# lbcb-sci/GNNome

Measured on AMD Instinct MI355X. Metric: edges/sec full-graph GatedGCN fwd, higher is better.
Workload: dtype f32

## Files before the change

### gnnome_amd/csrc/common.h

```cpp
#pragma once
#include <hip/hip_runtime.h>
#include <stdint.h>
#include <stdio.h>

#include "../../include/gnnome_hip.h"

namespace gnnome {

void set_error(const char* fmt, ...);

enum { kTuneGateVariant = 0, kTuneGateAblation = 1, kTuneLinearVariant = 2, kTuneGateTileOrder = 3, kTuneGateExperiment = 4, kTuneAggLdsKiB = 5, kTuneAggHubs = 6, kTuneAggVariant = 7, kTuneRefVariant = 8, kTuneOverlapBand = 9, kTuneArith = 10, kTuneCount = 16 };
int tuning(int key);

struct GateEnc {
    const float* e_raw;
    const int32_t* srt_eid;
    const float *W1, *b1, *W2, *b2;
    const float *W23, *b23;
};

struct GateBnBwd {
    const float *a, *c1, *c2, *mean, *rstd, *scale, *shift;
    float* a_out;
    int64_t n_once;
    unsigned* amax_bits = nullptr;
};

struct GateBfArgs {
    const float* e_in;
    float* e_out;
    int64_t E;
    const float* B1h;
    const float* B2h;
    int ldn;
    const int32_t* srt_src;
    const int32_t* srt_dst;
    const float* W3;
    int ldw;
    const float* scale;
    const float* shift;
    float* stats;
    int num_tiles;
    int abl;
    long long* prof;
    int xp;
    int num_cblocks, ld_out;
    GateEnc enc;
    GateBnBwd bnb;
};
int gate_bf_launch(int hidden, int mode, bool enc, const GateBfArgs& args, hipStream_t s, bool x16 = false, int extra = 0);
int gate_stream_launch(const float* e_in, float* e_out, int64_t E, const float* B1h, const float* B2h, int ldn, const int32_t* ss,
                       const int32_t* sd, const float* W3, int ldw, const float* scale, const float* shift, hipStream_t s);

int ws_linear_acc(const float* A, int64_t M, int K, const float* W, int ldw, float* C, hipStream_t s);
int stream_linear_acc_256(const float* A, int64_t M, const float* W, int ldw, float* C, hipStream_t s);
int gate_pl256_launch(int mode, const GateBfArgs& a, hipStream_t s, bool x16 = false);
int gate_f16_launch(int mode, const GateBfArgs& a, int grid, hipStream_t s, bool x16 = false);
int gate_enc256_launch(const GateBfArgs& a, hipStream_t s);
int gate_pl256_stats_rows();
void hub_cache_invalidate();
long long* gate_profile_buffer();
int linear_refm_launch(const float* A, int64_t M, int K, int lda, const float* W, int ldw, const float* bias, int Nout, float* C, int ldc,
                       hipStream_t s);
int gate_refm_launch(int hidden, bool with_enc, const float* e_in, float* e_out, int64_t E, const float* B1h, const float* B2h, int ldn,
                     const int32_t* ss, const int32_t* sd, const float* W3, int ldw, const float* b3, const float* scale, const float* shift,
                     const GateEnc& enc, hipStream_t s);

#define GN_REQUIRE(cond, ...)                 \
    do {                                      \
        if (!(cond)) {                        \
            ::gnnome::set_error(__VA_ARGS__); \
            return GNNOME_EINVAL;             \
        }                                     \
    } while (0)

#define GN_HIP(call)                                                                              \
    do {                                                                                          \
        hipError_t err__ = (call);                                                                \
        if (err__ != hipSuccess) {                                                                \
            ::gnnome::set_error("%s failed: %s (%s:%d)", #call, hipGetErrorString(err__), __FILE__, \
                                __LINE__);                                                        \
            return GNNOME_EHIP;                                                                   \
        }                                                                                         \
    } while (0)

#define GN_LAUNCH_CHECK() GN_HIP(hipGetLastError())

constexpr int kWave = 64;
constexpr int kXcds = 8;
constexpr int kNumCUs = 256;
int persistent_grid();
constexpr float kAggEps = 1e-6f;
constexpr float kNormEps = 1e-5f;

typedef float f32x4 __attribute__((ext_vector_type(4)));
typedef float f32x16 __attribute__((ext_vector_type(16)));

__device__ __forceinline__ unsigned bf16_bits(float x) {
    const unsigned u = __float_as_uint(x);
    return (u + 0x7FFFu + ((u >> 16) & 1u)) >> 16;
}
__device__ __forceinline__ uint2 pack_bf16x4(const f32x4 v) {
    return make_uint2(bf16_bits(v[0]) | (bf16_bits(v[1]) << 16), bf16_bits(v[2]) | (bf16_bits(v[3]) << 16));
}
__device__ __forceinline__ f32x4 unpack_bf16x4(const uint2 p) {
    return f32x4{__uint_as_float(p.x << 16), __uint_as_float(p.x & 0xFFFF0000u), __uint_as_float(p.y << 16),
                 __uint_as_float(p.y & 0xFFFF0000u)};
}
template <bool X16>
__device__ __forceinline__ f32x4 load4_as(const void* base, int64_t off) {
    if (X16) return unpack_bf16x4(*reinterpret_cast<const uint2*>(reinterpret_cast<const uint16_t*>(base) + off));
    return *reinterpret_cast<const f32x4*>(reinterpret_cast<const float*>(base) + off);
}
template <bool X16>
__device__ __forceinline__ void store4_as(void* base, int64_t off, const f32x4 v) {
    if (X16)
        *reinterpret_cast<uint2*>(reinterpret_cast<uint16_t*>(base) + off) = pack_bf16x4(v);
    else
        *reinterpret_cast<f32x4*>(reinterpret_cast<float*>(base) + off) = v;
}


__device__ __forceinline__ int xcd_remap(int bid, int n) {
    const int xcd = bid % kXcds, q = n / kXcds, r = n % kXcds;
    const int base = xcd < r ? xcd * (q + 1) : r * (q + 1) + (xcd - r) * q;
    return base + bid / kXcds;
}

__device__ __forceinline__ float sigmoidf_(float x) { return __builtin_amdgcn_rcpf(1.0f + __expf(-x)); }

__device__ __forceinline__ float relu_keep_nan(float t) { return t < 0.f ? 0.f : t; }

__device__ __forceinline__ void wave_amax_to(unsigned* amax_bits, float v) {
#pragma unroll
    for (int o = 32; o > 0; o >>= 1) v = fmaxf(v, __shfl_xor(v, o));
    if ((threadIdx.x & 63) == 0) {
        const unsigned b = __float_as_uint(v);
        if (b > __hip_atomic_load(amax_bits, __ATOMIC_RELAXED, __HIP_MEMORY_SCOPE_AGENT)) atomicMax(amax_bits, b);
    }
}

__device__ __forceinline__ float half_wave_sum(float v) {
    v += __shfl_xor(v, 1);
    v += __shfl_xor(v, 2);
    v += __shfl_xor(v, 4);
    v += __shfl_xor(v, 8);
    v += __shfl_xor(v, 16);
    return v;
}

}
```

### gnnome_amd/csrc/node_aggregate.hip

```cpp
#include "common.h"

#include <algorithm>
#include <map>
#include <mutex>
#include <utility>

namespace gnnome {

constexpr int kAggThreads = 256;
constexpr int kHubThreshold = 4096;
constexpr int kHubChunks = 128;
constexpr int kHubCap = 64;
constexpr int kHubMaxH = 256;
constexpr int kRecItems = 20;

struct HubScratch {
    const void *key_in = nullptr, *key_out = nullptr;
    int64_t key_n = -1;
    int* count = nullptr;
    int* nodes = nullptr;
    float* partials = nullptr;
    int* host_count = nullptr;
    hipEvent_t ready = nullptr;
    bool pending = false;
    int known = -1;
};

static std::map<std::pair<int, hipStream_t>, HubScratch> g_hub_table;
static std::mutex g_hub_guard;

void hub_cache_invalidate() {
    int dev = 0;
    if (hipGetDevice(&dev) != hipSuccess) return;
    std::lock_guard<std::mutex> lock(g_hub_guard);
    for (auto& kv : g_hub_table) {
        if (kv.first.first != dev) continue;
        kv.second.key_in = kv.second.key_out = nullptr;
        kv.second.key_n = -1;
        kv.second.known = -1;
        kv.second.pending = false;
    }
}

static HubScratch* hub_scratch(hipStream_t s, bool* capturing_unallocated, const void* in_ptr = nullptr, const void* out_ptr = nullptr,
                               int64_t n = -1) {
    int dev = 0;
    if (hipGetDevice(&dev) != hipSuccess) return nullptr;
    auto it = g_hub_table.find(std::make_pair(dev, s));
    if (it == g_hub_table.end() || it->second.partials == nullptr) {
        hipStreamCaptureStatus st = hipStreamCaptureStatusNone;
        if (hipStreamIsCapturing(s, &st) == hipSuccess && st != hipStreamCaptureStatusNone) {
            for (auto& kv : g_hub_table) {
                const HubScratch& h = kv.second;
                if (kv.first.first == dev && h.partials != nullptr && h.key_n == n &&
                    ((h.key_in == in_ptr && h.key_out == out_ptr) || (h.key_in == out_ptr && h.key_out == in_ptr)))
                    return &kv.second;
            }
            for (auto& kv : g_hub_table)
                if (kv.first.first == dev && kv.second.partials != nullptr) return &kv.second;
            *capturing_unallocated = true;
            return nullptr;
        }
    }
    HubScratch& h = g_hub_table[std::make_pair(dev, s)];
    if (h.partials == nullptr) {
        if (h.count == nullptr && hipMalloc(&h.count, sizeof(int) * (1 + kHubCap)) != hipSuccess) return nullptr;
        h.nodes = h.count + 1;
        if (hipMalloc(&h.partials, sizeof(float) * (size_t)kHubCap * kHubChunks * 4 * kHubMaxH) != hipSuccess) return nullptr;
        if (hipHostMalloc(&h.host_count, sizeof(int), hipHostMallocDefault) != hipSuccess) h.host_count = nullptr;
        if (h.host_count && hipEventCreateWithFlags(&h.ready, hipEventDisableTiming) != hipSuccess) h.ready = nullptr;
    }
    return &h;
}

__device__ __forceinline__ int hub_key(int node) { return 0x7fffffff - node; }
__device__ __forceinline__ int hub_node_at(const int* __restrict__ nodes, int slot) { return 0x7fffffff - nodes[slot]; }

__global__ __launch_bounds__(256) void k_find_hubs(const int32_t* __restrict__ in_ptr, const int32_t* __restrict__ out_ptr, int64_t n,
                                                   int* __restrict__ count, int* __restrict__ nodes) {
    const int64_t i = (int64_t)blockIdx.x * 256 + threadIdx.x;
    if (i >= n) return;
    const int cnt = (in_ptr[i + 1] - in_ptr[i]) + (out_ptr[i + 1] - out_ptr[i]);
    if (cnt > kHubThreshold) {
        atomicAdd(count, 1);
        int key = hub_key((int)i);
        if (key < __hip_atomic_load(nodes + kHubCap - 1, __ATOMIC_RELAXED, __HIP_MEMORY_SCOPE_AGENT)) return;
        for (int slot = 0; slot < kHubCap && key != 0; ++slot) {
            const int old = atomicMax(nodes + slot, key);
            key = min(old, key);
        }
    }
}

template <int H>
__device__ __forceinline__ float group_sum(float v) {
    constexpr int LPR = H / 4;
#pragma unroll
    for (int m = LPR; m < 64; m <<= 1) v += __shfl_xor(v, m);
    return v;
}

template <int H>
__device__ __forceinline__ float row_sum(float v) {
    constexpr int LPR = H / 4;
#pragma unroll
    for (int m = 1; m < LPR; m <<= 1) v += __shfl_xor(v, m);
    return v;
}

template <int H, int U = (H == 256 ? 8 : 4)>
__device__ __forceinline__ void accumulate_items(const float* __restrict__ e, const float* __restrict__ A2h, const float* __restrict__ A3h,
                                                 int ldn, const int32_t* __restrict__ srt_src, const int32_t* __restrict__ out_pos,
                                                 const int32_t* __restrict__ out_dst, int ib, int din, int ob, int lo, int hi, int lane,
                                                 int group, int c, f32x4& nf, f32x4& df, f32x4& nb, f32x4& db) {
    constexpr int LPR = H / 4, G = 64 / LPR;
    for (int base = lo; base < hi; base += 64) {
        const int j = base + lane;
        int my_p = 0, my_n = 0;
        if (j < din) {
            my_p = ib + j;
            my_n = srt_src[my_p];
        } else if (j < hi) {
            my_p = out_pos[ob + j - din];
            my_n = out_dst[ob + j - din];
        }
        const int m = min(64, hi - base);
        for (int j0 = 0; j0 < m; j0 += G * U) {
            f32x4 x[U], a[U];
            bool live[U], fwd[U];
#pragma unroll
            for (int u = 0; u < U; ++u) {
                const int item = j0 + u * G + group;
                live[u] = item < m;
                const int it = live[u] ? item : 0;
                const int p = __shfl(my_p, it), nn = __shfl(my_n, it);
                fwd[u] = base + it < din;
                const float* tb = fwd[u] ? A2h : A3h;
                x[u] = *reinterpret_cast<const f32x4*>(e + (int64_t)p * H + c);
                a[u] = *reinterpret_cast<const f32x4*>(tb + (int64_t)nn * ldn + c);
            }
#pragma unroll
            for (int u = 0; u < U; ++u) {
                if (live[u]) {
                    f32x4 s;
#pragma unroll
                    for (int k = 0; k < 4; ++k) s[k] = sigmoidf_(x[u][k]);
                    if (fwd[u]) {
                        nf += s * a[u];
                        df += s;
                    } else {
                        nb += s * a[u];
                        db += s;
                    }
                }
            }
        }
    }
}

template <int H, int U = (H == 256 ? 8 : 4), bool NOBR = false, bool NTOUT = false, bool TBLFIX = false>
__device__ __forceinline__ void accumulate_items_split(const float* __restrict__ e, const float* __restrict__ A2h, const float* __restrict__ A3h,
                                                       int ldn, const int32_t* __restrict__ srt_src, const int32_t* __restrict__ out_pos,
                                                       const int32_t* __restrict__ out_dst, int ib, int din, int ob, int lo, int hi, int lane,
                                                       int group, int c, f32x4& nf, f32x4& df, f32x4& nb, f32x4& db, int recv = 0,
                                                       bool rec_small = false) {
    constexpr int LPR = H / 4, G = 64 / LPR;
    for (int base = lo; base < hi; base += 64) {
        const int j = base + lane;
        int my_p = 0, my_n = 0;
        if (rec_small) {
            const int jo = min(max(j - din, 0), kRecItems - 1);
            my_n = __shfl(recv, j < din ? 4 + min(j, kRecItems - 1) : 4 + 2 * kRecItems + jo);
            my_p = __shfl(recv, 4 + kRecItems + jo);
        } else if (j < din) {
            my_n = srt_src[ib + j];
        } else if (j < hi) {
            my_p = out_pos[ob + j - din];
            my_n = out_dst[ob + j - din];
        }
        const int m = min(64, hi - base);
        const int m_in = min(m, max(din - base, 0));
        for (int j0 = 0; j0 < m_in; j0 += G * U) {
            f32x4 x[U], a[U];
            bool live[U];
#pragma unroll
            for (int u = 0; u < U; ++u) {
                const int item = j0 + u * G + group;
                live[u] = item < m_in;
                x[u] = *reinterpret_cast<const f32x4*>(e + (int64_t)(ib + base + (live[u] ? item : 0)) * H + c);
            }
#pragma unroll
            for (int u = 0; u < U; ++u) {
                const int item = j0 + u * G + group;
                const int nn = TBLFIX ? (ib & 1023) : __shfl(my_n, live[u] ? item : 0);
                a[u] = *reinterpret_cast<const f32x4*>(A2h + (int64_t)nn * ldn + c);
            }
#pragma unroll
            for (int u = 0; u < U; ++u) {
                if (NOBR) {
                    f32x4 s;
#pragma unroll
                    for (int k = 0; k < 4; ++k) s[k] = live[u] ? sigmoidf_(x[u][k]) : 0.f;
                    nf += s * a[u];
                    df += s;
                } else if (live[u]) {
                    f32x4 s;
#pragma unroll
                    for (int k = 0; k < 4; ++k) s[k] = sigmoidf_(x[u][k]);
                    nf += s * a[u];
                    df += s;
                }
            }
        }
        for (int j0 = m_in / (G * U) * (G * U); j0 < m; j0 += G * U) {
            f32x4 x[U], a[U];
            bool live[U];
#pragma unroll
            for (int u = 0; u < U; ++u) {
                const int item = j0 + u * G + group;
                live[u] = item >= m_in && item < m;
                const int it = live[u] ? item : m_in;
                const int p = __shfl(my_p, it), nn = TBLFIX ? (ib & 1023) : __shfl(my_n, it);
                x[u] = NTOUT ? __builtin_nontemporal_load(reinterpret_cast<const f32x4*>(e + (int64_t)p * H + c))
                             : *reinterpret_cast<const f32x4*>(e + (int64_t)p * H + c);
                a[u] = *reinterpret_cast<const f32x4*>(A3h + (int64_t)nn * ldn + c);
            }
#pragma unroll
            for (int u = 0; u < U; ++u) {
                if (NOBR) {
                    f32x4 s;
#pragma unroll
                    for (int k = 0; k < 4; ++k) s[k] = live[u] ? sigmoidf_(x[u][k]) : 0.f;
                    nb += s * a[u];
                    db += s;
                } else if (live[u]) {
                    f32x4 s;
#pragma unroll
                    for (int k = 0; k < 4; ++k) s[k] = sigmoidf_(x[u][k]);
                    nb += s * a[u];
                    db += s;
                }
            }
        }
    }
}

template <int H>
__global__ __launch_bounds__(kAggThreads) void k_hub_partials(const float* __restrict__ e, const float* __restrict__ A2h,
                                                              const float* __restrict__ A3h, int ldn, const int32_t* __restrict__ in_ptr,
                                                              const int32_t* __restrict__ srt_src, const int32_t* __restrict__ out_ptr,
                                                              const int32_t* __restrict__ out_pos, const int32_t* __restrict__ out_dst,
                                                              int64_t n_out, const int* __restrict__ hub_count,
                                                              const int* __restrict__ hub_nodes, float* __restrict__ partials) {
    constexpr int LPR = H / 4;
    const int lane = threadIdx.x & 63, wave = threadIdx.x >> 6;
    const int ch = blockIdx.x * (kAggThreads / 64) + wave;
    const int group = lane / LPR, c = (lane % LPR) * 4;
    const int nh = min(*hub_count, kHubCap);
    for (int h = 0; h < nh; ++h) {
        const int64_t node = hub_node_at(hub_nodes, h);
        if (node >= n_out) continue;
        const int ib = in_ptr[node], din = in_ptr[node + 1] - ib;
        const int ob = out_ptr[node], cnt = din + out_ptr[node + 1] - ob;
        const int per = ((cnt + kHubChunks - 1) / kHubChunks + 63) / 64 * 64;
        const int lo = min(cnt, ch * per), hi = min(cnt, lo + per);
        f32x4 nf = {0.f, 0.f, 0.f, 0.f}, df = nf, nb = nf, db = nf;
        accumulate_items<H>(e, A2h, A3h, ldn, srt_src, out_pos, out_dst, ib, din, ob, lo, hi, lane, group, c, nf, df, nb, db);
        f32x4 o0, o1, o2, o3;
#pragma unroll
        for (int k = 0; k < 4; ++k) {
            o0[k] = group_sum<H>(nf[k]);
            o1[k] = group_sum<H>(df[k]);
            o2[k] = group_sum<H>(nb[k]);
            o3[k] = group_sum<H>(db[k]);
        }
        if (group == 0) {
            float* pp = partials + ((int64_t)h * kHubChunks + ch) * 4 * H + c;
            *reinterpret_cast<f32x4*>(pp) = o0;
            *reinterpret_cast<f32x4*>(pp + H) = o1;
            *reinterpret_cast<f32x4*>(pp + 2 * H) = o2;
            *reinterpret_cast<f32x4*>(pp + 3 * H) = o3;
        }
    }
}

template <int H, int NORM, int MODE, bool HUBFIN = false, int U = (H == 256 ? 8 : 4), int WPS = 0, int SPLIT = 0, bool REC = false>
__global__ __launch_bounds__(kAggThreads, (WPS > 0 ? WPS : 1)) void k_node_aggregate(
    const float* __restrict__ e, int64_t n_out, const float* __restrict__ A1h, const float* __restrict__ A2h,
    const float* __restrict__ A3h, int ldn, const int32_t* __restrict__ in_ptr, const int32_t* __restrict__ srt_src,
    const int32_t* __restrict__ out_ptr, const int32_t* __restrict__ out_pos, const int32_t* __restrict__ out_dst,
    const float* __restrict__ h_in, int ldh, float* __restrict__ h_out, const float* __restrict__ scale,
    const float* __restrict__ shift, int total_blocks, float* __restrict__ aux0, float* __restrict__ aux1,
    float* __restrict__ aux2, float* __restrict__ aux3, const int* __restrict__ hub_count, const int* __restrict__ hub_nodes,
    const float* __restrict__ hub_partials, int64_t node0, int norm_width, const int32_t* __restrict__ records = nullptr) {
    constexpr int LPR = H / 4;
    const int lane = threadIdx.x & 63, wave = threadIdx.x >> 6;
    int64_t node;
    int hub_slot = -1;
    if (HUBFIN) {
        hub_slot = blockIdx.x * (kAggThreads / 64) + wave;
        if (hub_slot >= min(*hub_count, kHubCap)) return;
        node = hub_node_at(hub_nodes, hub_slot);
    } else {
        node = node0 + (int64_t)xcd_remap(blockIdx.x, total_blocks) * (kAggThreads / 64) + wave;
    }
    if (node >= n_out) return;
    const int group = lane / LPR, c = (lane % LPR) * 4;

    int ib, din, ob, cnt, recv = 0;
    if (REC) {
        recv = records[node * 64 + lane];
        ib = __builtin_amdgcn_readlane(recv, 0), din = __builtin_amdgcn_readlane(recv, 1);
        ob = __builtin_amdgcn_readlane(recv, 2), cnt = din + __builtin_amdgcn_readlane(recv, 3);
    } else {
        ib = in_ptr[node], din = in_ptr[node + 1] - ib;
        ob = out_ptr[node], cnt = din + out_ptr[node + 1] - ob;
    }
    const bool rec_small = REC && din <= kRecItems && cnt - din <= kRecItems;
    if (HUBFIN) {
        if (cnt <= kHubThreshold) return;
    } else if (cnt > kHubThreshold && hub_nodes != nullptr) {
        const int nh = min(*hub_count, kHubCap);
        bool listed = false;
        for (int base = 0; base < nh; base += 64) listed |= __ballot(base + lane < nh && hub_nodes[base + lane] == hub_key((int)node)) != 0;
        if (listed) return;
    }
    f32x4 a1 = {0.f, 0.f, 0.f, 0.f};
    if (MODE != 2) a1 = *reinterpret_cast<const f32x4*>(A1h + node * ldn + c);

    f32x4 nf = {0.f, 0.f, 0.f, 0.f}, df = nf, nb = nf, db = nf;
    if (HUBFIN) {
        if (group == 0) {
            const float* pp = hub_partials + ((int64_t)hub_slot * kHubChunks) * 4 * H + c;
            for (int ch = 0; ch < kHubChunks; ++ch, pp += 4 * H) {
                nf += *reinterpret_cast<const f32x4*>(pp);
                df += *reinterpret_cast<const f32x4*>(pp + H);
                nb += *reinterpret_cast<const f32x4*>(pp + 2 * H);
                db += *reinterpret_cast<const f32x4*>(pp + 3 * H);
            }
        }
    } else {
        if (SPLIT == 2)
            accumulate_items_split<H, U>(e, A2h, A3h, ldn, srt_src, out_pos, out_dst, ib, 0, ob, 0, cnt - din, lane, group, c, nf, df, nb, db);
        else if (SPLIT == 4)
            accumulate_items_split<H, U, false, true>(e, A2h, A3h, ldn, srt_src, out_pos, out_dst, ib, din, ob, 0, cnt, lane, group, c, nf, df, nb, db);
        else if (SPLIT == 5)
            accumulate_items_split<H, U, false, false, true>(e, A2h, A3h, ldn, srt_src, out_pos, out_dst, ib, din, ob, 0, cnt, lane, group, c, nf, df, nb, db);
        else if (SPLIT == 3)
            accumulate_items_split<H, U, true>(e, A2h, A3h, ldn, srt_src, out_pos, out_dst, ib, din, ob, 0, cnt, lane, group, c, nf, df, nb, db);
        else if (SPLIT == 1)
            accumulate_items_split<H, U>(e, A2h, A3h, ldn, srt_src, out_pos, out_dst, ib, din, ob, 0, cnt, lane, group, c, nf, df, nb, db, recv, rec_small);
        else
            accumulate_items<H, U>(e, A2h, A3h, ldn, srt_src, out_pos, out_dst, ib, din, ob, 0, cnt, lane, group, c, nf, df, nb, db);
    }

    f32x4 v, t0, t1, t2, t3;
#pragma unroll
    for (int k = 0; k < 4; ++k) {
        const float num_f = group_sum<H>(nf[k]), den_f = group_sum<H>(df[k]);
        const float num_b = group_sum<H>(nb[k]), den_b = group_sum<H>(db[k]);
        v[k] = a1[k] + num_f / (den_f + kAggEps) + num_b / (den_b + kAggEps);
        if (MODE == 1) {
            t0[k] = num_f / (den_f + kAggEps);
            t1[k] = 1.0f / (den_f + kAggEps);
            t2[k] = num_b / (den_b + kAggEps);
            t3[k] = 1.0f / (den_b + kAggEps);
        } else if (MODE == 2) {
            t0[k] = num_f;
            t2[k] = num_b;
        }
    }
    if (MODE != 0) {
        if (group == 0) {
            *reinterpret_cast<f32x4*>(aux0 + node * H + c) = t0;
            *reinterpret_cast<f32x4*>(aux2 + node * H + c) = t2;
            if (MODE == 1) {
                *reinterpret_cast<f32x4*>(aux1 + node * H + c) = t1;
                *reinterpret_cast<f32x4*>(aux3 + node * H + c) = t3;
                *reinterpret_cast<f32x4*>(h_out + node * H + c) = v;
            }
        }
        return;
    }
    if (NORM == GNNOME_NORM_LAYER) {
        const float inv_w = 1.0f / (float)norm_width;
        const float mean = row_sum<H>(v[0] + v[1] + v[2] + v[3]) * inv_w;
        float s2 = 0.f;
#pragma unroll
        for (int k = 0; k < 4; ++k) s2 += (c + k < norm_width) ? (v[k] - mean) * (v[k] - mean) : 0.f;
        const float rstd = rsqrtf(row_sum<H>(s2) * inv_w + kNormEps);
#pragma unroll
        for (int k = 0; k < 4; ++k) v[k] = (v[k] - mean) * rstd;
    }
    if (group == 0) {
        const f32x4 sc = *reinterpret_cast<const f32x4*>(scale + c);
        const f32x4 sh = *reinterpret_cast<const f32x4*>(shift + c);
        const f32x4 hi = *reinterpret_cast<const f32x4*>(h_in + node * ldh + c);
        f32x4 y;
#pragma unroll
        for (int k = 0; k < 4; ++k) y[k] = relu_keep_nan(v[k] * sc[k] + sh[k]) + hi[k];
        *reinterpret_cast<f32x4*>(h_out + node * H + c) = y;
    }
}

template <int NORM, int U = 4, bool PERSIST = false, bool NT = false>
__global__ __launch_bounds__(kAggThreads) void k_node_aggregate_pair(
    const float* __restrict__ e, int64_t n_out, const float* __restrict__ A1h, const float* __restrict__ A2h, const float* __restrict__ A3h,
    int ldn, const int32_t* __restrict__ in_ptr, const int32_t* __restrict__ srt_src, const int32_t* __restrict__ out_ptr,
    const int32_t* __restrict__ out_pos, const int32_t* __restrict__ out_dst, const float* __restrict__ h_in, int ldh,
    float* __restrict__ h_out, const float* __restrict__ scale, const float* __restrict__ shift, int total_blocks,
    const int* __restrict__ hub_count, const int* __restrict__ hub_nodes, int64_t node0) {
    constexpr int H = 128;
    const int lane = threadIdx.x & 63, wave = threadIdx.x >> 6, grp = lane >> 5, gl = lane & 31, c = 4 * gl;
    auto load_e = [&](int64_t row) {
        const f32x4* p = reinterpret_cast<const f32x4*>(e + row * H + c);
        return NT ? __builtin_nontemporal_load(p) : *p;
    };
    const int steps_per = PERSIST ? (total_blocks + (int)gridDim.x - 1) / (int)gridDim.x : 1;
    const int chunk = PERSIST ? xcd_remap(blockIdx.x, gridDim.x) : 0;
  for (int it = 0; it < steps_per; ++it) {
    const int64_t step = PERSIST ? (int64_t)chunk * steps_per + it : (int64_t)xcd_remap(blockIdx.x, total_blocks);
    if (PERSIST && step >= total_blocks) break;
    const int64_t node = node0 + 2 * (step * (kAggThreads / 64) + wave) + grp;
    bool valid = node < n_out;
    int ib = 0, din = 0, ob = 0, cnt = 0;
    if (valid) {
        ib = in_ptr[node], din = in_ptr[node + 1] - ib;
        ob = out_ptr[node], cnt = din + out_ptr[node + 1] - ob;
        if (cnt > kHubThreshold && hub_nodes != nullptr) {
            const int nh = min(*hub_count, kHubCap);
            for (int k = 0; k < nh; ++k) valid = valid && hub_nodes[k] != hub_key((int)node);
        }
    }
    if (!valid) cnt = din = 0;
    f32x4 a1 = {0.f, 0.f, 0.f, 0.f};
    if (valid) a1 = *reinterpret_cast<const f32x4*>(A1h + node * ldn + c);
    f32x4 nf = {0.f, 0.f, 0.f, 0.f}, df = nf, nb = nf, db = nf;
    const int cnt_w = max(__shfl(cnt, 0), __shfl(cnt, 32));
    for (int base = 0; base < cnt_w; base += 32) {
        const int j = base + gl;
        int my_p = 0, my_n = 0;
        if (j < din) {
            my_n = srt_src[ib + j];
        } else if (j < cnt) {
            my_p = out_pos[ob + j - din];
            my_n = out_dst[ob + j - din];
        }
        const int m = max(min(32, cnt - base), 0), m_in = min(m, max(din - base, 0));
        const int m_in_w = max(__shfl(m_in, 0), __shfl(m_in, 32)), m_out_w = max(__shfl(m - m_in, 0), __shfl(m - m_in, 32));
        for (int j0 = 0; j0 < m_in_w; j0 += U) {
            f32x4 x[U], a[U];
            bool live[U];
#pragma unroll
            for (int u = 0; u < U; ++u) {
                live[u] = j0 + u < m_in;
                x[u] = load_e((int64_t)(ib + base + (live[u] ? j0 + u : 0)));
            }
#pragma unroll
            for (int u = 0; u < U; ++u) {
                const int nn = __shfl(my_n, 32 * grp + (live[u] ? j0 + u : 0));
                a[u] = *reinterpret_cast<const f32x4*>(A2h + (int64_t)nn * ldn + c);
            }
#pragma unroll
            for (int u = 0; u < U; ++u) {
                f32x4 sg;
#pragma unroll
                for (int k = 0; k < 4; ++k) sg[k] = live[u] ? sigmoidf_(x[u][k]) : 0.f;
                nf += sg * a[u];
                df += sg;
            }
        }
        for (int j0 = 0; j0 < m_out_w; j0 += U) {
            f32x4 x[U], a[U];
            bool live[U];
#pragma unroll
            for (int u = 0; u < U; ++u) {
                const int item = m_in + j0 + u;
                live[u] = item < m;
                const int src_lane = 32 * grp + (live[u] ? item : (m > 0 ? m - 1 : 0));
                const int pp = __shfl(my_p, src_lane), nn = __shfl(my_n, src_lane);
                x[u] = load_e((int64_t)pp);
                a[u] = *reinterpret_cast<const f32x4*>(A3h + (int64_t)nn * ldn + c);
            }
#pragma unroll
            for (int u = 0; u < U; ++u) {
                f32x4 sg;
#pragma unroll
                for (int k = 0; k < 4; ++k) sg[k] = live[u] ? sigmoidf_(x[u][k]) : 0.f;
                nb += sg * a[u];
                db += sg;
            }
        }
    }
    if (!valid) continue;
    f32x4 v;
#pragma unroll
    for (int k = 0; k < 4; ++k) v[k] = a1[k] + nf[k] / (df[k] + kAggEps) + nb[k] / (db[k] + kAggEps);
    if (NORM == GNNOME_NORM_LAYER) {
        float s1 = v[0] + v[1] + v[2] + v[3];
#pragma unroll
        for (int o = 1; o < 32; o <<= 1) s1 += __shfl_xor(s1, o);
        const float mean = s1 * (1.0f / H);
        float s2 = 0.f;
#pragma unroll
        for (int k = 0; k < 4; ++k) s2 += (v[k] - mean) * (v[k] - mean);
#pragma unroll
        for (int o = 1; o < 32; o <<= 1) s2 += __shfl_xor(s2, o);
        const float rstd = rsqrtf(s2 * (1.0f / H) + kNormEps);
#pragma unroll
        for (int k = 0; k < 4; ++k) v[k] = (v[k] - mean) * rstd;
    }
    const f32x4 sc = *reinterpret_cast<const f32x4*>(scale + c), sh = *reinterpret_cast<const f32x4*>(shift + c);
    const f32x4 hi = *reinterpret_cast<const f32x4*>(h_in + node * ldh + c);
    f32x4 y;
#pragma unroll
    for (int k = 0; k < 4; ++k) y[k] = relu_keep_nan(v[k] * sc[k] + sh[k]) + hi[k];
    *reinterpret_cast<f32x4*>(h_out + node * H + c) = y;
  }
}

__global__ __launch_bounds__(256) void k_build_node_records(const int32_t* __restrict__ in_ptr, const int32_t* __restrict__ srt_src,
                                                            const int32_t* __restrict__ out_ptr, const int32_t* __restrict__ out_pos,
                                                            const int32_t* __restrict__ out_dst, int64_t n, int32_t* __restrict__ rec) {
    const int64_t t = (int64_t)blockIdx.x * 256 + threadIdx.x;
    const int64_t node = t >> 6;
    const int w = (int)(t & 63);
    if (node >= n) return;
    const int ib = in_ptr[node], din = in_ptr[node + 1] - ib, ob = out_ptr[node], dout = out_ptr[node + 1] - ob;
    int v = 0;
    if (w < 4) v = w == 0 ? ib : w == 1 ? din : w == 2 ? ob : dout;
    else if (w < 4 + kRecItems) v = (w - 4) < din ? srt_src[ib + w - 4] : 0;
    else if (w < 4 + 2 * kRecItems) v = (w - 4 - kRecItems) < dout ? out_pos[ob + w - 4 - kRecItems] : 0;
    else v = (w - 4 - 2 * kRecItems) < dout ? out_dst[ob + w - 4 - 2 * kRecItems] : 0;
    rec[t] = v;
}
static thread_local const int32_t* g_node_records = nullptr;

template <int H>
static int launch_agg(const float* e, int64_t n_out, const float* A1h, const float* A2h, const float* A3h, int ldn,
                      const int32_t* in_ptr, const int32_t* ss, const int32_t* out_ptr, const int32_t* out_pos,
                      const int32_t* od, const float* h_in, int ldh, float* h_out, int norm, const float* scale,
                      const float* shift, hipStream_t s, int mode = 0, float* aux0 = nullptr, float* aux1 = nullptr,
                      float* aux2 = nullptr, float* aux3 = nullptr, int64_t node_begin = 0, int64_t node_end = -1, int norm_width = 0) {
    if (norm_width <= 0) norm_width = H;
    if (node_end < 0) node_end = n_out;
    const int64_t node0 = node_begin;
    const int64_t blocks = (node_end - node_begin + (kAggThreads / 64) - 1) / (kAggThreads / 64);
    GN_REQUIRE(blocks < (1ll << 31), "node_aggregate: too many nodes");
    GN_REQUIRE(node_begin >= 0 && node_begin < node_end && node_end <= n_out, "node_aggregate: bad node range [%lld, %lld) of %lld",
               (long long)node_begin, (long long)node_end, (long long)n_out);
    bool capturing_unallocated = false;
    std::lock_guard<std::mutex> hub_lock(g_hub_guard);
    HubScratch* hub = tuning(kTuneAggHubs) == 1 ? nullptr : hub_scratch(s, &capturing_unallocated, in_ptr, out_ptr, n_out);
    GN_REQUIRE(!capturing_unallocated, "node_aggregate: first call on this device inside a stream capture - run one eager call first "
                                       "(the hub scratch is allocated on first use)");
    auto same_graph = [&](const HubScratch* h) {
        return h->key_n == n_out && ((h->key_in == in_ptr && h->key_out == out_ptr) || (h->key_in == out_ptr && h->key_out == in_ptr));
    };
    if (hub != nullptr && same_graph(hub)) {
        hipStreamCaptureStatus capq = hipStreamCaptureStatusNone;
        const bool capturing = hub->pending && (hipStreamIsCapturing(s, &capq) != hipSuccess || capq != hipStreamCaptureStatusNone);
        if (hub->pending && !capturing && hipEventQuery(hub->ready) == hipSuccess) {
            hub->known = *hub->host_count;
            hub->pending = false;
        }
        if (hub->known == 0) hub = nullptr;
    }
    const bool hub_pass = hub != nullptr && node_begin == 0;
    const int* hub_count = hub ? hub->count : nullptr;
    const int* hub_nodes = hub ? hub->nodes : nullptr;
    const float* hub_partials = hub ? hub->partials : nullptr;
    if (hub && !hub_pass)
        GN_REQUIRE(same_graph(hub), "node_aggregate_range: the ranges of one aggregation must start with the range that begins at node 0");
    if (hub_pass) {
        if (!same_graph(hub)) {
            GN_HIP(hipMemsetAsync(hub->count, 0, sizeof(int) * (1 + kHubCap), s));
            hipLaunchKernelGGL(k_find_hubs, dim3((unsigned)((n_out + 255) / 256)), dim3(256), 0, s, in_ptr, out_ptr, n_out, hub->count, hub->nodes);
            hub->key_in = in_ptr, hub->key_out = out_ptr, hub->key_n = n_out;
            hub->known = -1, hub->pending = false;
            hipStreamCaptureStatus cap = hipStreamCaptureStatusNone;
            if (hub->ready != nullptr && hipStreamIsCapturing(s, &cap) == hipSuccess && cap == hipStreamCaptureStatusNone) {
                if (hipMemcpyAsync(hub->host_count, hub->count, sizeof(int), hipMemcpyDeviceToHost, s) == hipSuccess &&
                    hipEventRecord(hub->ready, s) == hipSuccess)
                    hub->pending = true;
            }
        }
        hipLaunchKernelGGL((k_hub_partials<H>), dim3(kHubChunks / (kAggThreads / 64)), dim3(kAggThreads), 0, s, e, A2h, A3h, ldn, in_ptr, ss, out_ptr,
                           out_pos, od, n_out, hub->count, hub->nodes, hub->partials);
    }
    const size_t dyn = (size_t)tuning(kTuneAggLdsKiB) * 1024;
#define GN_AGG_LAUNCH_S(NORM_, MODE_, FIN_, U_, WPS_, GRID_, SPLIT_)                                                                           \
    hipLaunchKernelGGL((k_node_aggregate<H, NORM_, MODE_, FIN_, U_, WPS_, SPLIT_>), dim3((unsigned)(GRID_)), dim3(kAggThreads), (FIN_) ? 0 : dyn, s, e, \
                       (FIN_) ? n_out : node_end, A1h, A2h, A3h, ldn, in_ptr, ss, out_ptr, out_pos, od, h_in, ldh, h_out, scale, shift,   \
                       (int)blocks, aux0, aux1, aux2, aux3, hub_count, hub_nodes, hub_partials, (FIN_) ? (int64_t)0 : node0, norm_width)
#define GN_AGG_LAUNCH(NORM_, MODE_, FIN_, U_, WPS_, GRID_) GN_AGG_LAUNCH_S(NORM_, MODE_, FIN_, U_, WPS_, GRID_, 1)
    constexpr int UD = H == 256 ? 2 : 4;
    constexpr int kFinGrid = kHubCap / (kAggThreads / 64);
    if (mode == 1) {
        GN_AGG_LAUNCH(GNNOME_NORM_AFFINE, 1, false, UD, 0, blocks);
        if (hub_pass) GN_AGG_LAUNCH(GNNOME_NORM_AFFINE, 1, true, UD, 0, kFinGrid);
    } else if (mode == 2) {
        GN_AGG_LAUNCH(GNNOME_NORM_AFFINE, 2, false, UD, 0, blocks);
        if (hub_pass) GN_AGG_LAUNCH(GNNOME_NORM_AFFINE, 2, true, UD, 0, kFinGrid);
    } else if (norm == GNNOME_NORM_AFFINE) {
        switch (tuning(kTuneAggVariant)) {
            case 1: GN_AGG_LAUNCH(GNNOME_NORM_AFFINE, 0, false, 4, 8, blocks); break;
            case 2: GN_AGG_LAUNCH(GNNOME_NORM_AFFINE, 0, false, 2, 8, blocks); break;
            case 3: GN_AGG_LAUNCH(GNNOME_NORM_AFFINE, 0, false, 1, 0, blocks); break;
            case 4: GN_AGG_LAUNCH(GNNOME_NORM_AFFINE, 0, false, 8, 0, blocks); break;
            case 5: GN_AGG_LAUNCH(GNNOME_NORM_AFFINE, 0, false, 2, 0, blocks); break;
            case 6: GN_AGG_LAUNCH_S(GNNOME_NORM_AFFINE, 0, false, UD, 0, blocks, 0); break;
            case 7: GN_AGG_LAUNCH_S(GNNOME_NORM_AFFINE, 0, false, UD, 0, blocks, 2); break;
            case 8: GN_AGG_LAUNCH_S(GNNOME_NORM_AFFINE, 0, false, UD, 0, blocks, 3); break;
            case 14: GN_AGG_LAUNCH_S(GNNOME_NORM_AFFINE, 0, false, UD, 0, blocks, 4); break;
            case 15: GN_AGG_LAUNCH_S(GNNOME_NORM_AFFINE, 0, false, UD, 0, blocks, 5); break;
            case 11:
            case 12:
            case 13:
                if (H == 128) {
                    const int64_t pblocks = ((node_end - node_begin + 1) / 2 + (kAggThreads / 64) - 1) / (kAggThreads / 64);
                    const int per_cu = tuning(kTuneAggVariant) == 13 ? 8 : 4;
                    const unsigned pgrid = (unsigned)std::min<int64_t>(pblocks, (int64_t)persistent_grid() * per_cu);
                    if (tuning(kTuneAggVariant) == 11)
                        hipLaunchKernelGGL((k_node_aggregate_pair<GNNOME_NORM_AFFINE, 4, true, false>), dim3(pgrid), dim3(kAggThreads), dyn, s, e, node_end, A1h, A2h, A3h, ldn,
                                           in_ptr, ss, out_ptr, out_pos, od, h_in, ldh, h_out, scale, shift, (int)pblocks, hub_count, hub_nodes, node0);
                    else
                        hipLaunchKernelGGL((k_node_aggregate_pair<GNNOME_NORM_AFFINE, 4, true, true>), dim3(pgrid), dim3(kAggThreads), dyn, s, e, node_end, A1h, A2h, A3h, ldn,
                                           in_ptr, ss, out_ptr, out_pos, od, h_in, ldh, h_out, scale, shift, (int)pblocks, hub_count, hub_nodes, node0);
                } else {
                    GN_AGG_LAUNCH(GNNOME_NORM_AFFINE, 0, false, UD, 0, blocks);
                }
                break;
            case 9:
            case 10:
                if (H == 128) {
                    const int64_t pblocks = ((node_end - node_begin + 1) / 2 + (kAggThreads / 64) - 1) / (kAggThreads / 64);
                    if (tuning(kTuneAggVariant) == 9)
                        hipLaunchKernelGGL((k_node_aggregate_pair<GNNOME_NORM_AFFINE, 4>), dim3((unsigned)pblocks), dim3(kAggThreads), dyn, s, e, node_end, A1h, A2h, A3h, ldn,
                                           in_ptr, ss, out_ptr, out_pos, od, h_in, ldh, h_out, scale, shift, (int)pblocks, hub_count, hub_nodes, node0);
                    else
                        hipLaunchKernelGGL((k_node_aggregate_pair<GNNOME_NORM_AFFINE, 2>), dim3((unsigned)pblocks), dim3(kAggThreads), dyn, s, e, node_end, A1h, A2h, A3h, ldn,
                                           in_ptr, ss, out_ptr, out_pos, od, h_in, ldh, h_out, scale, shift, (int)pblocks, hub_count, hub_nodes, node0);
                } else {
                    GN_AGG_LAUNCH(GNNOME_NORM_AFFINE, 0, false, UD, 0, blocks);
                }
                break;
            default:
                if (g_node_records != nullptr && node_begin == 0 && node_end == n_out)
                    hipLaunchKernelGGL((k_node_aggregate<H, GNNOME_NORM_AFFINE, 0, false, UD, 0, 1, true>), dim3((unsigned)blocks), dim3(kAggThreads), dyn, s, e, node_end,
                                       A1h, A2h, A3h, ldn, in_ptr, ss, out_ptr, out_pos, od, h_in, ldh, h_out, scale, shift, (int)blocks, aux0, aux1, aux2, aux3,
                                       hub_count, hub_nodes, hub_partials, node0, norm_width, g_node_records);
                else
                    GN_AGG_LAUNCH(GNNOME_NORM_AFFINE, 0, false, UD, 0, blocks);
                break;
        }
        if (hub_pass) GN_AGG_LAUNCH(GNNOME_NORM_AFFINE, 0, true, UD, 0, kFinGrid);
    } else {
        GN_AGG_LAUNCH(GNNOME_NORM_LAYER, 0, false, UD, 0, blocks);
        if (hub_pass) GN_AGG_LAUNCH(GNNOME_NORM_LAYER, 0, true, UD, 0, kFinGrid);
    }
#undef GN_AGG_LAUNCH
#undef GN_AGG_LAUNCH_S
    GN_LAUNCH_CHECK();
    return GNNOME_OK;
}

}

extern "C" int gnnome_build_node_records(const int32_t* in_ptr, const int32_t* srt_src, const int32_t* out_ptr, const int32_t* out_pos,
                                         const int32_t* out_dst, int64_t num_nodes, int32_t* records, void* stream) {
    using namespace gnnome;
    GN_REQUIRE(num_nodes >= 0 && num_nodes < (1ll << 25), "build_node_records: node count out of range");
    if (num_nodes == 0) return GNNOME_OK;
    GN_REQUIRE(in_ptr && out_ptr && records && (uintptr_t)records % 256 == 0, "build_node_records: null or misaligned pointer");
    hipLaunchKernelGGL(k_build_node_records, dim3((unsigned)((num_nodes * 64 + 255) / 256)), dim3(256), 0, (hipStream_t)stream, in_ptr, srt_src, out_ptr,
                       out_pos, out_dst, num_nodes, records);
    GN_LAUNCH_CHECK();
    return GNNOME_OK;
}
extern "C" int gnnome_debug_node_records(const int32_t* records) {
    gnnome::g_node_records = records;
    return GNNOME_OK;
}

extern "C" int gnnome_node_aggregate_f32(const float* e, int hidden, int64_t num_nodes_out, const float* A1h,
                                         const float* A2h, const float* A3h, int ld_node, const int32_t* in_ptr,
                                         const int32_t* srt_src, const int32_t* out_ptr, const int32_t* out_pos,
                                         const int32_t* out_dst, const float* h_in, int ld_h, float* h_out,
                                         int norm_kind, const float* norm_scale, const float* norm_shift, void* stream) {
    using namespace gnnome;
    GN_REQUIRE(num_nodes_out >= 0, "node_aggregate: negative node count");
    if (num_nodes_out == 0) return GNNOME_OK;
    GN_REQUIRE(A1h && A2h && A3h && in_ptr && out_ptr && h_in && h_out && norm_scale && norm_shift,
               "node_aggregate: null pointer");
    const int norm_width = (norm_kind >> 8) ? (norm_kind >> 8) : hidden;
    norm_kind &= 0xFF;
    GN_REQUIRE(norm_width >= 1 && norm_width <= hidden && (norm_width == hidden || norm_kind == GNNOME_NORM_LAYER), "node_aggregate: bad norm width %d", norm_width);
    GN_REQUIRE(norm_kind == GNNOME_NORM_AFFINE || norm_kind == GNNOME_NORM_LAYER, "node_aggregate: bad norm_kind %d",
               norm_kind);
    GN_REQUIRE(ld_node >= hidden && ld_node % 4 == 0 && ld_h >= hidden && ld_h % 4 == 0, "node_aggregate: bad strides");
    GN_REQUIRE(((uintptr_t)A1h % 16 == 0) && ((uintptr_t)A2h % 16 == 0) && ((uintptr_t)A3h % 16 == 0) &&
                   ((uintptr_t)h_in % 16 == 0) && ((uintptr_t)h_out % 16 == 0) && ((uintptr_t)e % 16 == 0),
               "node_aggregate: tensors must be 16-byte aligned");
    hipStream_t s = (hipStream_t)stream;
    switch (hidden) {
        case 64: return launch_agg<64>(e, num_nodes_out, A1h, A2h, A3h, ld_node, in_ptr, srt_src, out_ptr, out_pos, out_dst, h_in, ld_h, h_out, norm_kind, norm_scale, norm_shift, s, 0, nullptr, nullptr, nullptr, nullptr, 0, -1, norm_width);
        case 128: return launch_agg<128>(e, num_nodes_out, A1h, A2h, A3h, ld_node, in_ptr, srt_src, out_ptr, out_pos, out_dst, h_in, ld_h, h_out, norm_kind, norm_scale, norm_shift, s, 0, nullptr, nullptr, nullptr, nullptr, 0, -1, norm_width);
        case 256: return launch_agg<256>(e, num_nodes_out, A1h, A2h, A3h, ld_node, in_ptr, srt_src, out_ptr, out_pos, out_dst, h_in, ld_h, h_out, norm_kind, norm_scale, norm_shift, s, 0, nullptr, nullptr, nullptr, nullptr, 0, -1, norm_width);
        default: set_error("node_aggregate: hidden=%d not in {64,128,256}", hidden); return GNNOME_EINVAL;
    }
}

extern "C" int gnnome_node_aggregate_range_f32(const float* e, int hidden, int64_t num_nodes_out, int64_t node_begin, int64_t node_end,
                                               const float* A1h, const float* A2h, const float* A3h, int ld_node, const int32_t* in_ptr,
                                               const int32_t* srt_src, const int32_t* out_ptr, const int32_t* out_pos,
                                               const int32_t* out_dst, const float* h_in, int ld_h, float* h_out, int norm_kind,
                                               const float* norm_scale, const float* norm_shift, void* stream) {
    using namespace gnnome;
    GN_REQUIRE(num_nodes_out > 0, "node_aggregate_range: empty graph");
    GN_REQUIRE(A1h && A2h && A3h && in_ptr && out_ptr && h_in && h_out && norm_scale && norm_shift, "node_aggregate_range: null pointer");
    const int norm_width = (norm_kind >> 8) ? (norm_kind >> 8) : hidden;
    norm_kind &= 0xFF;
    GN_REQUIRE(norm_width >= 1 && norm_width <= hidden && (norm_width == hidden || norm_kind == GNNOME_NORM_LAYER), "node_aggregate_range: bad norm width %d", norm_width);
    GN_REQUIRE(norm_kind == GNNOME_NORM_AFFINE || norm_kind == GNNOME_NORM_LAYER, "node_aggregate_range: bad norm_kind %d", norm_kind);
    GN_REQUIRE(ld_node >= hidden && ld_node % 4 == 0 && ld_h >= hidden && ld_h % 4 == 0, "node_aggregate_range: bad strides");
    GN_REQUIRE(((uintptr_t)A1h % 16 == 0) && ((uintptr_t)A2h % 16 == 0) && ((uintptr_t)A3h % 16 == 0) &&
                   ((uintptr_t)h_in % 16 == 0) && ((uintptr_t)h_out % 16 == 0) && ((uintptr_t)e % 16 == 0),
               "node_aggregate_range: tensors must be 16-byte aligned");
    hipStream_t s = (hipStream_t)stream;
    switch (hidden) {
        case 64: return launch_agg<64>(e, num_nodes_out, A1h, A2h, A3h, ld_node, in_ptr, srt_src, out_ptr, out_pos, out_dst, h_in, ld_h, h_out, norm_kind, norm_scale, norm_shift, s, 0, nullptr, nullptr, nullptr, nullptr, node_begin, node_end, norm_width);
        case 128: return launch_agg<128>(e, num_nodes_out, A1h, A2h, A3h, ld_node, in_ptr, srt_src, out_ptr, out_pos, out_dst, h_in, ld_h, h_out, norm_kind, norm_scale, norm_shift, s, 0, nullptr, nullptr, nullptr, nullptr, node_begin, node_end, norm_width);
        case 256: return launch_agg<256>(e, num_nodes_out, A1h, A2h, A3h, ld_node, in_ptr, srt_src, out_ptr, out_pos, out_dst, h_in, ld_h, h_out, norm_kind, norm_scale, norm_shift, s, 0, nullptr, nullptr, nullptr, nullptr, node_begin, node_end, norm_width);
        default: set_error("node_aggregate_range: hidden=%d not in {64,128,256}", hidden); return GNNOME_EINVAL;
    }
}

extern "C" int gnnome_node_aggregate_raw_f32(const float* e, int hidden, int64_t num_nodes, int mode, const float* A1h,
                                             const float* A2h, const float* A3h, int ld_node, const int32_t* in_ptr,
                                             const int32_t* srt_src, const int32_t* out_ptr, const int32_t* out_pos,
                                             const int32_t* out_dst, float* v_out, float* aux0, float* aux1, float* aux2,
                                             float* aux3, void* stream) {
    using namespace gnnome;
    GN_REQUIRE(num_nodes >= 0 && (mode == 1 || mode == 2), "node_aggregate_raw: mode must be 1 or 2");
    if (num_nodes == 0) return GNNOME_OK;
    GN_REQUIRE(A2h && A3h && in_ptr && out_ptr && aux0 && aux2 && ld_node >= hidden && ld_node % 4 == 0, "node_aggregate_raw: bad arguments");
    GN_REQUIRE(mode == 2 || (A1h && v_out && aux1 && aux3), "node_aggregate_raw: mode 1 needs A1h, v_out, aux1, aux3");
    hipStream_t s = (hipStream_t)stream;
    switch (hidden) {
        case 64: return launch_agg<64>(e, num_nodes, A1h, A2h, A3h, ld_node, in_ptr, srt_src, out_ptr, out_pos, out_dst, nullptr, hidden, v_out, 0, nullptr, nullptr, s, mode, aux0, aux1, aux2, aux3);
        case 128: return launch_agg<128>(e, num_nodes, A1h, A2h, A3h, ld_node, in_ptr, srt_src, out_ptr, out_pos, out_dst, nullptr, hidden, v_out, 0, nullptr, nullptr, s, mode, aux0, aux1, aux2, aux3);
        case 256: return launch_agg<256>(e, num_nodes, A1h, A2h, A3h, ld_node, in_ptr, srt_src, out_ptr, out_pos, out_dst, nullptr, hidden, v_out, 0, nullptr, nullptr, s, mode, aux0, aux1, aux2, aux3);
        default: set_error("node_aggregate_raw: hidden=%d not in {64,128,256}", hidden); return GNNOME_EINVAL;
    }
}
```

Measured before the change: 236.1 million.

## Add lean aggregation loop with 32-bit row addressing and packed sigmoid

```diff
diff --git a/gnnome_amd/csrc/common.h b/gnnome_amd/csrc/common.h
--- a/gnnome_amd/csrc/common.h
+++ b/gnnome_amd/csrc/common.h
@@ -9,7 +9,7 @@
 
 void set_error(const char* fmt, ...);
 
-enum { kTuneGateVariant = 0, kTuneGateAblation = 1, kTuneLinearVariant = 2, kTuneGateTileOrder = 3, kTuneGateExperiment = 4, kTuneAggLdsKiB = 5, kTuneAggHubs = 6, kTuneAggVariant = 7, kTuneRefVariant = 8, kTuneOverlapBand = 9, kTuneArith = 10, kTuneCount = 16 };
+enum { kTuneGateVariant = 0, kTuneGateAblation = 1, kTuneLinearVariant = 2, kTuneGateTileOrder = 3, kTuneGateExperiment = 4, kTuneAggLdsKiB = 5, kTuneAggHubs = 6, kTuneAggVariant = 7, kTuneRefVariant = 8, kTuneOverlapBand = 9, kTuneArith = 10, kTuneAggAddr64 = 11, kTuneCount = 16 };
 int tuning(int key);
 
 struct GateEnc {
@@ -129,6 +129,18 @@
 
 __device__ __forceinline__ float sigmoidf_(float x) { return __builtin_amdgcn_rcpf(1.0f + __expf(-x)); }
 
+typedef float f32x2 __attribute__((ext_vector_type(2)));
+__device__ __forceinline__ f32x2 packed_(f32x2 v) {
+    asm("" : "+v"(v));
+    return v;
+}
+__device__ __forceinline__ f32x4 sigmoid4_(const f32x4 x) {
+    const f32x2 t0 = packed_(packed_(f32x2{x[0], x[1]}) * -1.4426950408889634f), t1 = packed_(packed_(f32x2{x[2], x[3]}) * -1.4426950408889634f);
+    const f32x2 d0 = packed_(packed_(f32x2{__builtin_amdgcn_exp2f(t0[0]), __builtin_amdgcn_exp2f(t0[1])}) + 1.0f);
+    const f32x2 d1 = packed_(packed_(f32x2{__builtin_amdgcn_exp2f(t1[0]), __builtin_amdgcn_exp2f(t1[1])}) + 1.0f);
+    return f32x4{__builtin_amdgcn_rcpf(d0[0]), __builtin_amdgcn_rcpf(d0[1]), __builtin_amdgcn_rcpf(d1[0]), __builtin_amdgcn_rcpf(d1[1])};
+}
+
 __device__ __forceinline__ float relu_keep_nan(float t) { return t < 0.f ? 0.f : t; }
 
 __device__ __forceinline__ void wave_amax_to(unsigned* amax_bits, float v) {
diff --git a/gnnome_amd/csrc/node_aggregate.hip b/gnnome_amd/csrc/node_aggregate.hip
--- a/gnnome_amd/csrc/node_aggregate.hip
+++ b/gnnome_amd/csrc/node_aggregate.hip
@@ -239,6 +239,105 @@
                     for (int k = 0; k < 4; ++k) s[k] = sigmoidf_(x[u][k]);
                     nb += s * a[u];
                     db += s;
+                }
+            }
+        }
+    }
+}
+
+__device__ __forceinline__ int opaque_(int v) {
+    asm volatile("" : "+v"(v));
+    return v;
+}
+
+template <int H, int U = (H == 256 ? 8 : 4)>
+__device__ __forceinline__ void accumulate_items_lean(const float* __restrict__ e, const float* __restrict__ A2h, const float* __restrict__ A3h,
+                                                      int ldn, const int32_t* __restrict__ srt_src, const int32_t* __restrict__ out_pos,
+                                                      const int32_t* __restrict__ out_dst, int ib, int din, int ob, int lo, int hi, int lane,
+                                                      int group, int c, f32x4& nf, f32x4& df, f32x4& nb, f32x4& db, uint32_t a32_rows) {
+    constexpr int LPR = H / 4, G = 64 / LPR;
+    constexpr uint32_t kPosLimit = (uint32_t)((1ull << 32) / (H * 4));
+    const uint32_t lc = (uint32_t)c * 4, lg = (uint32_t)group * (H * 4) + lc;
+    auto pick = [&](uint32_t v, int it) -> uint32_t {
+        if (G == 1) return (uint32_t)__builtin_amdgcn_readlane((int)v, __builtin_amdgcn_readfirstlane(it));
+        return (uint32_t)__builtin_amdgcn_ds_bpermute(it << 2, (int)v);
+    };
+    auto row32 = [&](const float* tb, uint32_t off) -> f32x4 {
+        return *reinterpret_cast<const f32x4*>(reinterpret_cast<const char*>(tb) + (size_t)(uint32_t)(off + lc));
+    };
+    auto row64 = [&](const float* tb, uint32_t idx, int stride) -> f32x4 { return *reinterpret_cast<const f32x4*>(tb + (int64_t)(int)idx * stride + c); };
+    for (int base = lo; base < hi; base += 64) {
+        const int j = base + lane;
+        int my_p = 0, my_n = 0;
+        if (j < din) {
+            my_n = srt_src[ib + j];
+        } else if (j < hi) {
+            my_p = out_pos[ob + j - din];
+            my_n = out_dst[ob + j - din];
+        }
+        const int m = min(64, hi - base);
+        const int m_in = min(m, max(din - base, 0));
+        for (int j0 = 0; j0 < m_in; j0 += G * U) {
+            const char* xb = reinterpret_cast<const char*>(e + (int64_t)(ib + base + j0) * H);
+            f32x4 x[U], a[U];
+            bool live[U];
+#pragma unroll
+            for (int u = 0; u < U; ++u) {
+                live[u] = j0 + u * G + group < m_in;
+                x[u] = *reinterpret_cast<const f32x4*>(xb + (size_t)(live[u] ? lg + (uint32_t)(u * G * H * 4) : lc));
+            }
+            const uint32_t nn = (uint32_t)opaque_(my_n);
+            if (__ballot(nn >= a32_rows) == 0) {
+                const uint32_t no = nn * (uint32_t)(ldn * 4);
+#pragma unroll
+                for (int u = 0; u < U; ++u) a[u] = row32(A2h, pick(no, live[u] ? j0 + u * G + group : j0));
+            } else {
+#pragma unroll
+                for (int u = 0; u < U; ++u) a[u] = row64(A2h, pick(nn, live[u] ? j0 + u * G + group : j0), ldn);
+            }
+#pragma unroll
+            for (int u = 0; u < U; ++u) {
+                if (live[u]) {
+                    const f32x4 s = sigmoid4_(x[u]);
+                    nf += s * a[u];
+                    df += s;
+                }
+            }
+        }
+        if (m_in < m) {
+            const uint32_t pp = (uint32_t)my_p, nn = (uint32_t)my_n;
+            const bool fit = __ballot(pp >= kPosLimit || nn >= a32_rows) == 0;
+            const uint32_t po = pp * (uint32_t)(H * 4), no = nn * (uint32_t)(ldn * 4);
+            for (int j0 = m_in / (G * U) * (G * U); j0 < m; j0 += G * U) {
+                f32x4 x[U], a[U];
+                bool live[U];
+                int it[U];
+#pragma unroll
+                for (int u = 0; u < U; ++u) {
+                    const int item = j0 + u * G + group;
+                    live[u] = item >= m_in && item < m;
+                    it[u] = live[u] ? item : m_in;
+                }
+                if (fit) {
+#pragma unroll
+                    for (int u = 0; u < U; ++u) {
+                        x[u] = row32(e, pick(po, it[u]));
+                        a[u] = row32(A3h, pick(no, it[u]));
+                    }
+                } else {
+#pragma unroll
+                    for (int u = 0; u < U; ++u) {
+                        x[u] = row64(e, pick(pp, it[u]), H);
+                        a[u] = row64(A3h, pick(nn, it[u]), ldn);
+                    }
+                }
+#pragma unroll
+                for (int u = 0; u < U; ++u) {
+                    if (live[u]) {
+                        const f32x4 s = sigmoid4_(x[u]);
+                        nb += s * a[u];
+                        db += s;
+                    }
                 }
             }
         }
@@ -292,9 +391,10 @@
     const float* __restrict__ h_in, int ldh, float* __restrict__ h_out, const float* __restrict__ scale,
     const float* __restrict__ shift, int total_blocks, float* __restrict__ aux0, float* __restrict__ aux1,
     float* __restrict__ aux2, float* __restrict__ aux3, const int* __restrict__ hub_count, const int* __restrict__ hub_nodes,
-    const float* __restrict__ hub_partials, int64_t node0, int norm_width, const int32_t* __restrict__ records = nullptr) {
+    const float* __restrict__ hub_partials, int64_t node0, int norm_width, const int32_t* __restrict__ records = nullptr,
+    uint32_t a32_rows = 0) {
     constexpr int LPR = H / 4;
-    const int lane = threadIdx.x & 63, wave = threadIdx.x >> 6;
+    const int lane = threadIdx.x & 63, wave = SPLIT == 6 ? __builtin_amdgcn_readfirstlane(threadIdx.x >> 6) : threadIdx.x >> 6;
     int64_t node;
     int hub_slot = -1;
     if (HUBFIN) {
@@ -348,6 +448,8 @@
             accumulate_items_split<H, U, false, false, true>(e, A2h, A3h, ldn, srt_src, out_pos, out_dst, ib, din, ob, 0, cnt, lane, group, c, nf, df, nb, db);
         else if (SPLIT == 3)
             accumulate_items_split<H, U, true>(e, A2h, A3h, ldn, srt_src, out_pos, out_dst, ib, din, ob, 0, cnt, lane, group, c, nf, df, nb, db);
+        else if (SPLIT == 6)
+            accumulate_items_lean<H, U>(e, A2h, A3h, ldn, srt_src, out_pos, out_dst, ib, din, ob, 0, cnt, lane, group, c, nf, df, nb, db, a32_rows);
         else if (SPLIT == 1)
             accumulate_items_split<H, U>(e, A2h, A3h, ldn, srt_src, out_pos, out_dst, ib, din, ob, 0, cnt, lane, group, c, nf, df, nb, db, recv, rec_small);
         else
@@ -592,9 +694,18 @@
 #define GN_AGG_LAUNCH_S(NORM_, MODE_, FIN_, U_, WPS_, GRID_, SPLIT_)                                                                           \
     hipLaunchKernelGGL((k_node_aggregate<H, NORM_, MODE_, FIN_, U_, WPS_, SPLIT_>), dim3((unsigned)(GRID_)), dim3(kAggThreads), (FIN_) ? 0 : dyn, s, e, \
                        (FIN_) ? n_out : node_end, A1h, A2h, A3h, ldn, in_ptr, ss, out_ptr, out_pos, od, h_in, ldh, h_out, scale, shift,   \
-                       (int)blocks, aux0, aux1, aux2, aux3, hub_count, hub_nodes, hub_partials, (FIN_) ? (int64_t)0 : node0, norm_width)
-#define GN_AGG_LAUNCH(NORM_, MODE_, FIN_, U_, WPS_, GRID_) GN_AGG_LAUNCH_S(NORM_, MODE_, FIN_, U_, WPS_, GRID_, 1)
+                       (int)blocks, aux0, aux1, aux2, aux3, hub_count, hub_nodes, hub_partials, (FIN_) ? (int64_t)0 : node0, norm_width, nullptr, a32_rows)
+#define GN_AGG_LAUNCH(NORM_, MODE_, FIN_, U_, WPS_, GRID_)                                \
+    do {                                                                                  \
+        constexpr int kLoop = (!(FIN_) && (WPS_) == 0 && (U_) == UD) ? 6 : 1;             \
+        if (kLoop == 6 && prev_loop)                                                      \
+            GN_AGG_LAUNCH_S(NORM_, MODE_, FIN_, U_, WPS_, GRID_, 1);                      \
+        else                                                                              \
+            GN_AGG_LAUNCH_S(NORM_, MODE_, FIN_, U_, WPS_, GRID_, kLoop);                  \
+    } while (0)
     constexpr int UD = H == 256 ? 2 : 4;
+    const bool prev_loop = tuning(kTuneAggVariant) == 16;
+    const uint32_t a32_rows = tuning(kTuneAggAddr64) == 1 ? 0u : (uint32_t)((1ull << 32) / ((uint64_t)ldn * 4));
     constexpr int kFinGrid = kHubCap / (kAggThreads / 64);
     if (mode == 1) {
         GN_AGG_LAUNCH(GNNOME_NORM_AFFINE, 1, false, UD, 0, blocks);
```

Measured after the change: 239.1 million, median of 6. 1.01x the previous value.
